# msracver/Relation-Networks-for-Object-Detection

Hardware: AMD Instinct MI355X
Metric: images/sec (1000x600, 300 ROIs) (higher is better)
Workload: dtype bf16; 1 GPU; BASELINE configs[1]: ResNet-101 Faster-RCNN + 2 relation modules (N=300, 16 heads, d=1024) + soft-NMS(0.6) + top-100, 600x1000 images, 300 proposals, random-init weights; launch=hipGraph replay, batches_in_flight=1, parallelism=replicas x1 (no data-path collective), ranks_seen_by_rccl=1

## Files before the change

### include/relnet_hip.h

```cpp
#ifndef RELNET_HIP_H
#define RELNET_HIP_H

#ifdef __cplusplus
extern "C" {
#endif

enum { RELNET_F32 = 0, RELNET_BF16 = 1 };

int relnet_version(void);
const char* relnet_last_error(void);
unsigned long long relnet_stream_capture_id(void* stream);

void _nms(int* keep_out, int* num_out, const float* boxes_host, int boxes_num, int boxes_dim,
          float nms_overlap_thresh, int device_id);

int relnet_proposal_decode(const float* cls_prob, const long* cls_strides4, const float* deltas,
                           const long* delta_strides4, const float* im_info, const double* base_anchors,
                           float* boxes , float* scores , int B, int A, int h, int w,
                           int feat_stride, int min_size, int softmax_pairs, void* stream);
int relnet_topk_sort(const float* scores, const float* boxes, float* out_boxes5, int* out_index,
                     int* out_count, int B, int n, int K, void* stream);
int relnet_nms_mask(const float* boxes5, const int* counts , unsigned long long* mask,
                    int B, int n, int n_stride, float thresh, void* stream);
int relnet_nms_scan(const unsigned long long* mask, const float* boxes5, const int* counts, float* rois,
// ... 89 lines not shown
                                 int B, int H, int N, int M, int Mpad, float scale, int in_dtype, int out_dtype,
                                 const int* key_count, void* stream);
void relnet_relation_attention_debug_lds_f32(int on);

int relnet_relation_attention_fused(const void* q, long q_ld, long q_bs, const void* k, long k_ld, long k_bs,
                                    const void* vwt, long vwt_ld, long vwt_bs, const float* boxes, int box_stride,
                                    int box_off, const float* wp, const float* bp, const float* divisors8,
                                    const float* bout, const void* resid, long resid_ld, long resid_bs, void* out,
                                    long out_ld, long out_bs, void* out_act, long act_ld, long act_bs, int B, int H,
                                    int N, int M, int Mpad, float scale, void* stream);

int relnet_bottleneck_chain(const void* mid2, const void* x, const void* w3f, const void* w1f, const float* b3,
                            const float* b1, void* x_next, void* mid1_next, long P, int mid, void* stream);
int relnet_bottleneck_chain_proj(const void* mid2, const void* x_in, const void* w3f, const void* wpf, const void* w1f,
                                 const float* b3p, const float* b1, void* x_next, void* mid1_next, long P, int mid, void* stream);

int relnet_conv3x3_c64(const void* in, const void* w_frag, const float* bias, int relu, void* out, int B, int H, int W,
                       void* stream);


int relnet_pack_w_frag(const void* w, long ldw, void* out, int N, int K, void* stream);
int relnet_conv2d_nhwc_wf(const void* in, long in_pix, long in_img, const void* w, const void* w_frag, const float* bias,
                          const void* resid, int relu, void* out, long ldc, int B, int H, int W, int Cin, int Cout, int R,
                          int S, int stride, int dil, int pad, int out_dtype, void* stream);

int relnet_detect_head(const float* cls_score, long cs_ld, const float* bbox_pred, long bp_ld, const float* rois,
                       const float* im_info, float* cls_prob, double* boxes, int R, int C, int rois_per_image,
                       int delta_off, void* stream);
int relnet_detect_head_ex(const float* cls_score, long cs_ld, const float* bbox_pred, long bp_ld, const float* rois,
                          const float* im_info, float* cls_prob, double* boxes, int R, int C, int rois_per_image,
                          int delta_off, const int* n_valid, void* stream);
int relnet_class_nms(const float* cls_prob, const double* boxes, double* dets, int* counts, int B, int N, int C,
                     float score_thresh, double nms_param, int soft, int max_picks, void* stream);
// ... 227 lines not shown
```

### relation-networks-for-object-detection_amd/backbone.py

```python
import math
import os

import torch
import torch.nn.functional as F

from . import ops

UNITS = (3, 4, 23, 3)
FILTERS = (256, 512, 1024, 2048)
EPS = 1e-5
PIXEL_MEANS = (103.06, 115.90, 123.15)


def unit_names(fpn=False):
    out = []
    in_ch = 64
    for si, (n, oc) in enumerate(zip(UNITS, FILTERS)):
        stage = si + 2
        for u in range(n):
            if n <= 3 or stage == 2 or stage == 5:
                name = 'abc'[u]
            else:
                name = 'a' if u == 0 else 'b%d' % u
            stride = 2 if (u == 0 and (stage in (3, 4) or (fpn and stage == 5))) else 1
# ... 67 lines not shown


class Backbone(object):

    def __init__(self, params, dtype=torch.bfloat16, device='cuda', channels_last=True, impl=None, stem='hip', dcn=False,
                 fpn=False, chain=True, frozen_only=False, pixel_means=PIXEL_MEANS):
        self.dtype, self.device, self.dcn, self.fpn = dtype, device, dcn, fpn
        self.frozen_only = frozen_only
        self.pixel_means = tuple(float(v) for v in pixel_means)
        self.use_chain = chain
        env = os.environ.get('RELNET_STAGE_SPLIT')
        if env not in (None, '', '0'):
            self.stage_split = {int(a): int(b) for a, b in (kv.split(':') for kv in env.split(','))}
        if os.environ.get('RELNET_INPLACE_EXPAND') is not None:
            self.inplace_expand = os.environ['RELNET_INPLACE_EXPAND'] not in ('', '0')
        self.impl = impl or ('hip' if dtype == torch.bfloat16 else ('hip32' if dtype == torch.float32 and torch.device(device).type == 'cuda' else 'miopen'))
        if self.impl == 'hip' and torch.device(device).type == 'cuda':
            ops.asm_selfcheck()
        self.stem = stem
        assert self.impl in ('hip', 'hip32', 'miopen') and (self.impl != 'hip' or dtype == torch.bfloat16) and (self.impl != 'hip32' or dtype == torch.float32)
        self.mf = torch.channels_last if channels_last else torch.contiguous_format
        self.w = {}
        self.wp = {}
        self.wf = {}
        self.b32 = {}
        self.wp32 = {}
        for conv, bn, oc, ic, k in conv_bn_names():
            if frozen_only and not conv.startswith(('conv1', 'res2')):
                continue
            w, b = fold_bn(params[conv + '_weight'], params[bn + '_gamma'], params[bn + '_beta'],
# ... 90 lines not shown
    def _forward_hip(self, data, rpn_hook=None, im_info=None):
        if self.stem == 'hip':
            x = ops.stem_fused(data, self.w_stem, self.b32['conv1'], im_info, self.pixel_means)
        elif self.stem == 'hip3':
            x = ops.stem_conv7(self._float_image(data, im_info, torch.float32), self.w_stem, self.b32['conv1'], relu=True)
            x = ops.stem_bias_relu_pool(x, self.zero_bias64)
        else:
            x = self._float_image(data, im_info, torch.float32).to(self.dtype).contiguous(memory_format=self.mf)
            x = F.conv2d(x, self.w['conv1'][0], None, stride=2, padding=3)
            x = ops.stem_bias_relu_pool(x.permute(0, 2, 3, 1), self.b32['conv1'])
        conv4 = None
        ends = {}
        y_next = None
        side, hooked = None, None
        self.last_chain_units, self.last_side_stream, self.last_stage_split = [], False, {}
        ui = 0
        while ui < len(self.units):
            unit = self.units[ui]
            stage, proj = unit[0], unit[7]
            if stage == 5 and conv4 is None:
                conv4 = x
                if rpn_hook is not None and not self.fpn:
                    main = torch.cuda.current_stream()
                    side = self._side_stream()
                    self.last_side_stream = True
                    side.wait_stream(main)
                    with torch.cuda.stream(side):
                        hooked = self._rpn_head(conv4)
                        hooked = hooked + (rpn_hook(hooked[0], hooked[1]),)
            if proj and stage > 2:
                ends[stage - 1] = x
            nsplit = self._stage_split(stage, x, unit) if proj else 1
            if nsplit > 1:
                stage_units = [u for u in self.units if u[0] == stage]
                x = self._run_stage_split(x, stage_units, nsplit)
                ui += len(stage_units)
                continue
            x, y_next = self._unit_hip(x, unit, y_next, inplace=self.inplace_expand)
            ui += 1
        conv5 = x
        nchw = lambda t: t.permute(0, 3, 1, 2)
        if self.fpn:
            tops = {32: self._hconv(conv5, 'fpn_ft32_1x1')}
            for lvl, src in ((16, ends[4]), (8, ends[3]), (4, ends[2])):
                tops[lvl] = ops.upsample2x_add_(self._hconv(src, 'fpn_ft%d_1x1' % lvl), tops[lvl * 2])
            out = {'fpn_ft%d' % lvl: nchw(self._hconv(tops[lvl], 'fpn_ft%d_3x3' % lvl, pad=1)) for lvl in (4, 8, 16, 32)}
            out.update(conv4=nchw(conv4), conv5=nchw(conv5))
            return out
        feat = self._hconv(conv5, 'conv_new_1', relu=True)
        out = dict(conv4=nchw(conv4), conv5=nchw(conv5), conv_new_1_relu=nchw(feat))
        if hooked is not None:
            torch.cuda.current_stream().wait_stream(side)
            out.update(rpn_cls_score=hooked[0], rpn_bbox_pred=hooked[1], rpn_hook=hooked[2])
        else:
            out['rpn_cls_score'], out['rpn_bbox_pred'] = self._rpn_head(conv4)
        return out

    stage_split = None
    inplace_expand = True

    def _stage_split(self, stage, x, unit):
        return int(self.stage_split.get(stage, 1)) if self.stage_split else 1

    def _run_stage_split(self, x, stage_units, nsplit):
        B = x.shape[0]
        stage = stage_units[0][0]
        st, nm, ic, mc, oc, stride, dil, proj = stage_units[0]
        Ho, Wo = (x.shape[1] - 1) // stride + 1, (x.shape[2] - 1) // stride + 1
        out = torch.empty((B, Ho, Wo, oc), device=x.device, dtype=x.dtype)
        bounds = [(B * i) // nsplit for i in range(nsplit + 1)]
        self.last_stage_split[stage] = [hi - lo for lo, hi in zip(bounds, bounds[1:])]
        for lo, hi in zip(bounds, bounds[1:]):
            xs, ys = x[lo:hi], None
            for unit in stage_units:
                xs, ys = self._unit_hip(xs, unit, ys, sc_out=out[lo:hi] if unit[7] else None, inplace=self.inplace_expand, force_chain=True)
            if xs.data_ptr() != out[lo:hi].data_ptr():
                out[lo:hi].copy_(xs)
        return out

    def _unit_hip(self, x, unit, y_pre=None, sc_out=None, inplace=False, force_chain=False):
        stage, nm, ic, mc, oc, stride, dil, proj = unit
        fuse_proj = (nm in self.chain_proj and sc_out is None and x.is_contiguous()
                     and (force_chain or ops.chain_worthwhile(x.numel() // x.shape[-1], mc)))
        if fuse_proj:
            sc = None
        elif proj:
            w, b, k = self.wp['res%s_branch1' % nm]
            sc = ops.conv2d_nhwc(x, w, b, ksize=k, stride=stride, out=sc_out)
        else:
            sc = x
        y = y_pre if y_pre is not None else self._hconv(x, 'res%s_branch2a' % nm, stride=stride, relu=True)
        if self.dcn and stage == 5:
            y = self._deform_2b(y.permute(0, 3, 1, 2), 'res%s_branch2b' % nm,
                                self._hconv(y, 'res%s_branch2b_offset' % nm, pad=2, dil=2, out_dtype=torch.float32).permute(0, 3, 1, 2))
            y = y.permute(0, 2, 3, 1)
        elif ('res%s_branch2b' % nm) in self.halo3:
# ... 117 lines not shown
```

### relation-networks-for-object-detection_amd/csrc/bottleneck.hip

```cpp
#include "common.h"

namespace relnet {

typedef const __attribute__((address_space(1))) void* gas_ptr;
typedef __attribute__((address_space(3))) void* las_ptr;

__device__ __forceinline__ void chain_glds16(const void* src, unsigned lds_byte_addr) {
  asm volatile("s_mov_b32 m0, %1\n\ts_nop 0\n\tglobal_load_lds_dwordx4 %0, off" ::"v"(src), "s"(lds_byte_addr) : "memory", "m0");
}

struct ChainArgs {
  const unsigned short* m2;
  const unsigned short* x;
  const uint4* w3f;
  const uint4* w1f;
  const float* b3;
  const float* b1;
  const unsigned short* xin;
  const uint4* wpf;
  unsigned short* xn;
  unsigned short* m1;
  int P;
  int dbg;
};

template <int MID, bool STREAM, bool REDUCE = true, int KSPLIT = 1, bool PROJ = false>
__global__ __launch_bounds__(512) void bottleneck_chain_kernel(ChainArgs a) {
  static_assert(!PROJ || (!STREAM && KSPLIT == 1), "the projection form exists for the resident-weight kernel");
  static_assert(KSPLIT == 1 || (STREAM && !REDUCE), "k-split passes exist for the streamed expand-only form");
  constexpr int COUT = 4 * MID, KS = MID / 16, KSS = KS / KSPLIT, RT = MID / 32, NP = COUT / 64;
  static_assert(!REDUCE || MID <= 128, "MID = 256 with the second product is chain256_roles_kernel");
  constexpr int W3P = 2 * KSS * 1024, W1P = REDUCE ? 4 * RT * 1024 : 0;
  constexpr int WPP = PROJ ? W3P : 0;
  constexpr int PASSB = W3P + WPP + W1P;
  constexpr int STG = PROJ ? 4096 : 8192;
  constexpr int WBYTES = STREAM ? 2 * PASSB : NP * PASSB;
  extern __shared__ __attribute__((aligned(16))) unsigned char smem[];
  const int tid = threadIdx.x, lane = tid & 63;
  const int wave = __builtin_amdgcn_readfirstlane(tid >> 6);
  const int half = lane >> 5, l31 = lane & 31;
  unsigned char* stage = smem + WBYTES + wave * STG;
  float* sB3 = (float*)(smem + WBYTES + 8 * STG);
  float* sB1 = sB3 + COUT;
  for (int i = tid; i < COUT; i += 512) sB3[i] = a.b3[i];
  if constexpr (REDUCE) for (int i = tid; i < MID; i += 512) sB1[i] = a.b1[i];
  if constexpr (!STREAM) {
    for (int i = tid; i < NP * PASSB / 16; i += 512) {
      const int p = i / (PASSB / 16), r = i % (PASSB / 16);
      uint4 v;
      if (r < W3P / 16) v = a.w3f[(long)p * (W3P / 16) + r];
      else if (r < (W3P + WPP) / 16) v = a.wpf[(long)p * (W3P / 16) + (r - W3P / 16)];
      else { const int q = (r - (W3P + WPP) / 16) >> 6, rt = q >> 2, kk = q & 3; v = a.w1f[((long)rt * (COUT / 16) + p * 4 + kk) * 64 + (r & 63)]; }
      ((uint4*)smem)[i] = v;
    }
  }
  __syncthreads();
  const int ntile = (a.P + 31) / 32;
  const int drow = lane >> 3, dslot = lane & 7;
  auto issue_x = [&](int p0, int p) {
    if constexpr (PROJ) return;
    unsigned char* sb = stage + (p & 1) * 4096;
#pragma unroll
    for (int i = 0; i < 4; ++i) {
      const int row = 8 * i + drow;
      const unsigned off = ((unsigned)min(p0 + row, a.P - 1) * COUT + p * 64 + ((dslot ^ ((row >> 1) & 7)) << 3)) * 2u;
      __builtin_amdgcn_global_load_lds((gas_ptr)((const unsigned char*)a.x + off), (las_ptr)(sb + i * 1024), 16, 0, 0);
    }
  };
  auto issue_w = [&](int st) {
    if constexpr (STREAM) {
      const int p = st / KSPLIT, kh = st % KSPLIT;
      unsigned char* wb = smem + (st & 1) * PASSB;
#pragma unroll
      for (int i = 0; i < (2 * KSS + (REDUCE ? 4 * RT : 0)) / 8; ++i) {
        const int q = wave + 8 * i;
        if (q < 2 * KSS) {
          const int ct = q / KSS, ks = q % KSS;
          __builtin_amdgcn_global_load_lds((gas_ptr)(a.w3f + ((long)((p * 2 + ct) * KS + kh * KSS + ks) * 64 + lane)), (las_ptr)(wb + q * 1024), 16, 0, 0);
        } else {
          const int q1 = q - 2 * KSS, rt = q1 >> 2, kk = q1 & 3;
// ... 6 lines not shown
    const unsigned char* sb = stage + (PROJ ? 0 : (p & 1) * 4096) + lane * 16;
    const uint4 v0 = *(const uint4*)sb, v1 = *(const uint4*)(sb + 1024), v2 = *(const uint4*)(sb + 2048), v3 = *(const uint4*)(sb + 3072);
    asm volatile("s_waitcnt lgkmcnt(0)" ::: "memory");
    auto put = [&](int i, const uint4& v) {
      const int row = 8 * i + drow;
      if (p0 + row < a.P) *(uint4*)((unsigned char*)a.xn + ((unsigned)(p0 + row) * COUT + p * 64 + ((dslot ^ ((row >> 1) & 7)) << 3)) * 2u) = v;
    };
    put(0, v0); put(1, v1); put(2, v2); put(3, v3);
  };

  const int t_first = blockIdx.x * 8 + wave;
  const int t_step = gridDim.x * 8;
  const int n_iter = STREAM ? ((ntile + 7) / 8 - (int)blockIdx.x + (int)gridDim.x - 1) / (int)gridDim.x
                            : (ntile - t_first + t_step - 1) / t_step;
  if (n_iter <= 0) return;
  issue_x(t_first * 32, 0);
  issue_w(0);
  for (int it = 0; it < n_iter; ++it) {
    const int p0 = (t_first + it * t_step) * 32;
    const int px = min(p0 + l31, a.P - 1);
    bf16x8 m2f[KS];
#pragma unroll
    for (int ks = 0; ks < KS; ++ks) m2f[ks] = *(const bf16x8*)(a.m2 + (long)px * MID + 16 * ks + 8 * half);
    bf16x8 xf[PROJ ? KS : 1];
    if constexpr (PROJ) {
#pragma unroll
      for (int ks = 0; ks < KS; ++ks) xf[ks] = *(const bf16x8*)(a.xin + (long)px * MID + 16 * ks + 8 * half);
    }
    f32x16 m1acc[RT];
#pragma unroll
    for (int rt = 0; rt < RT; ++rt)
#pragma unroll
      for (int r = 0; r < 16; ++r) m1acc[rt][r] = 0.f;
#pragma unroll 1
    for (int p = 0; p < NP; ++p) {
      f32x16 acc[2];
#pragma unroll
      for (int kh = 0; kh < KSPLIT; ++kh) {
        const int st = p * KSPLIT + kh;
        if constexpr (STREAM) asm volatile("s_waitcnt vmcnt(0)\n\ts_barrier" ::: "memory");
        else if constexpr (!PROJ) asm volatile("s_waitcnt vmcnt(0)" ::: "memory");
        if (kh == 0) {
          if (!PROJ && p > 0) flush(p0, p - 1);
          if (p + 1 < NP) issue_x(p0, p + 1);
          else if (it + 1 < n_iter) issue_x(p0 + t_step * 32, 0);
        }
        if (st + 1 < NP * KSPLIT) issue_w(st + 1);
        else if (it + 1 < n_iter) issue_w(0);
        const uint4* w3 = (const uint4*)(smem + (STREAM ? (st & 1) : st) * PASSB);
#pragma unroll
        for (int ct = 0; ct < 2; ++ct) {
          if (kh == 0)
#pragma unroll
            for (int r = 0; r < 16; ++r) acc[ct][r] = 0.f;
#pragma unroll
          for (int ks = 0; ks < KSS; ++ks)
            acc[ct] = __builtin_amdgcn_mfma_f32_32x32x16_bf16(*(const bf16x8*)&w3[(ct * KSS + ks) * 64 + lane], m2f[kh * KSS + ks], acc[ct], 0, 0, 0);
          if constexpr (PROJ) {
            const uint4* wp = (const uint4*)((const unsigned char*)w3 + W3P);
#pragma unroll
// ... 260 lines not shown
using namespace relnet;

static int g_chain_dbg = 0;
extern "C" void relnet_chain_debug(int flags) { g_chain_dbg = flags; }

extern "C" int relnet_bottleneck_chain(const void* mid2, const void* x, const void* w3f, const void* w1f, const float* b3,
                                       const float* b1, void* x_next, void* mid1_next, long P, int mid, void* stream) {
  RELNET_REQUIRE(mid2 && x && w3f && b3 && x_next, "relnet_bottleneck_chain: null operand");
  RELNET_REQUIRE((w1f && b1 && mid1_next) || (!w1f && !b1 && !mid1_next), "relnet_bottleneck_chain: w1f, b1 and mid1_next are given together (or all NULL: expand + shortcut + ReLU only)");
  RELNET_REQUIRE(mid == 64 || mid == 128 || mid == 256 || (mid == 512 && !mid1_next), "relnet_bottleneck_chain: mid = %d unsupported (64, 128, 256; 512 without the reduce product)", mid);
  RELNET_REQUIRE(P > 0 && P * 8 * mid < (1L << 32), "relnet_bottleneck_chain: bad pixel count %ld (the 4 mid-channel map must stay below 4 GiB)", P);
  ChainArgs a;
  a.m2 = (const unsigned short*)mid2; a.x = (const unsigned short*)x; a.w3f = (const uint4*)w3f; a.w1f = (const uint4*)w1f;
  a.b3 = b3; a.b1 = b1; a.xn = (unsigned short*)x_next; a.m1 = (unsigned short*)mid1_next; a.P = (int)P;
  a.xin = nullptr; a.wpf = nullptr; a.dbg = g_chain_dbg;
  static relnet::PerDeviceOnce attr_once;
  if (attr_once.first()) {
    hipFuncSetAttribute((const void*)bottleneck_chain_kernel<64, false>, hipFuncAttributeMaxDynamicSharedMemorySize, 160 * 1024);
    hipFuncSetAttribute((const void*)bottleneck_chain_kernel<128, true>, hipFuncAttributeMaxDynamicSharedMemorySize, 160 * 1024);
    hipFuncSetAttribute((const void*)bottleneck_chain_kernel<64, false, false>, hipFuncAttributeMaxDynamicSharedMemorySize, 160 * 1024);
    hipFuncSetAttribute((const void*)bottleneck_chain_kernel<128, true, false>, hipFuncAttributeMaxDynamicSharedMemorySize, 160 * 1024);
    hipFuncSetAttribute((const void*)bottleneck_chain_kernel<256, true, false>, hipFuncAttributeMaxDynamicSharedMemorySize, 160 * 1024);
    hipFuncSetAttribute((const void*)bottleneck_chain_kernel<512, true, false, 2>, hipFuncAttributeMaxDynamicSharedMemorySize, 160 * 1024);
    hipFuncSetAttribute((const void*)chain256_roles_kernel, hipFuncAttributeMaxDynamicSharedMemorySize, 160 * 1024);
  }
  const long ntile = (P + 31) / 32;
  const unsigned grid = (unsigned)(ntile < 8 * 256 ? (ntile + 7) / 8 : 256);
  const size_t lds = 65536  + 65536  + (size_t)5 * mid * 4;
  if (mid1_next) {
    if (mid == 64) bottleneck_chain_kernel<64, false><<<grid, 512, lds, (hipStream_t)stream>>>(a);
    else if (mid == 128) bottleneck_chain_kernel<128, true><<<grid, 512, lds, (hipStream_t)stream>>>(a);
    else {
      const long nset = (ntile + 3) / 4;
      chain256_roles_kernel<<<(unsigned)(nset < 256 ? nset : 256), 512, relnet::kRolesLdsBytes, (hipStream_t)stream>>>(a);
    }
  } else {
    if (mid == 64) bottleneck_chain_kernel<64, false, false><<<grid, 512, lds, (hipStream_t)stream>>>(a);
    else if (mid == 128) bottleneck_chain_kernel<128, true, false><<<grid, 512, lds, (hipStream_t)stream>>>(a);
    else if (mid == 256) bottleneck_chain_kernel<256, true, false><<<grid, 512, lds, (hipStream_t)stream>>>(a);
    else bottleneck_chain_kernel<512, true, false, 2><<<grid, 512, lds, (hipStream_t)stream>>>(a);
  }
  return check_launch("relnet_bottleneck_chain");
}

extern "C" int relnet_bottleneck_chain_proj(const void* mid2, const void* x_in, const void* w3f, const void* wpf, const void* w1f,
                                            const float* b3p, const float* b1, void* x_next, void* mid1_next, long P, int mid,
                                            void* stream) {
  RELNET_REQUIRE(mid2 && x_in && w3f && wpf && b3p && x_next, "relnet_bottleneck_chain_proj: null operand");
  RELNET_REQUIRE((w1f && b1 && mid1_next) || (!w1f && !b1 && !mid1_next), "relnet_bottleneck_chain_proj: w1f, b1 and mid1_next are given together (or all NULL)");
  RELNET_REQUIRE(mid == 64, "relnet_bottleneck_chain_proj: mid = %d unsupported (64)", mid);
  RELNET_REQUIRE(P > 0 && P * 8 * mid < (1L << 32), "relnet_bottleneck_chain_proj: bad pixel count %ld (x_next is addressed with 32-bit byte offsets: the 4 mid-channel map must stay below 4 GiB)", P);
  ChainArgs a;
  a.m2 = (const unsigned short*)mid2; a.x = nullptr; a.w3f = (const uint4*)w3f; a.w1f = (const uint4*)w1f;
  a.b3 = b3p; a.b1 = b1; a.xn = (unsigned short*)x_next; a.m1 = (unsigned short*)mid1_next; a.P = (int)P;
  a.xin = (const unsigned short*)x_in; a.wpf = (const uint4*)wpf; a.dbg = 0;
  static relnet::PerDeviceOnce attr_once;
  if (attr_once.first()) {
    hipFuncSetAttribute((const void*)bottleneck_chain_kernel<64, false, true, 1, true>, hipFuncAttributeMaxDynamicSharedMemorySize, 160 * 1024);
    hipFuncSetAttribute((const void*)bottleneck_chain_kernel<64, false, false, 1, true>, hipFuncAttributeMaxDynamicSharedMemorySize, 160 * 1024);
  }
  const long ntile = (P + 31) / 32;
  const unsigned grid = (unsigned)(ntile < 8 * 256 ? (ntile + 7) / 8 : 256);
  const size_t lds = (size_t)4 * (8192 + 8192 + (mid1_next ? 8192 : 0)) + 8 * 4096 + (size_t)5 * mid * 4;
  if (mid1_next) bottleneck_chain_kernel<64, false, true, 1, true><<<grid, 512, lds, (hipStream_t)stream>>>(a);
  else bottleneck_chain_kernel<64, false, false, 1, true><<<grid, 512, lds, (hipStream_t)stream>>>(a);
  return check_launch("relnet_bottleneck_chain_proj");
}

namespace relnet {

__device__ __attribute__((aligned(16))) const unsigned int g_zero_chunk[4] = {0u, 0u, 0u, 0u};

struct Halo3Args {
  const unsigned short* in;
  const uint4* wf;
  const float* bias;
  unsigned short* out;
  int B, H, W, relu;
  int tiles_x, tiles_y;
};

constexpr int kHaloW = 34, kHaloSlots = 40;
constexpr int kHaloBytes = 10 * kHaloSlots * 128;

__global__ __launch_bounds__(512) void conv3x3_c64_halo_kernel(Halo3Args a) {
  extern __shared__ __attribute__((aligned(16))) unsigned char smem[];
  unsigned char* sOut = smem + 2 * kHaloBytes;
  const int tid = threadIdx.x, lane = tid & 63;
  const int wave = __builtin_amdgcn_readfirstlane(tid >> 6);
  const int half = lane >> 5, l31 = lane & 31;
  const int chh = wave & 1, rg = wave >> 1;
  bf16x8 wfrag[36];
#pragma unroll
  for (int ks = 0; ks < 36; ++ks) wfrag[ks] = *(const bf16x8*)&a.wf[(chh * 36 + ks) * 64 + lane];
  float* sBias = (float*)(sOut + 32768);
  if (tid < 64) sBias[tid] = a.bias[tid];
  const int per_img = a.tiles_x * a.tiles_y;
  const int ntile = a.B * per_img;

  auto issue_halo = [&](int t, unsigned char* buf) {
    asm volatile("" : "+s"(t));
    const int b = t / per_img, ty = (t % per_img) / a.tiles_x, tx = t % a.tiles_x;
    const int y0 = ty * 8 - 1, x0 = tx * 32 - 1;
    const unsigned short* img = a.in + (long)b * a.H * a.W * 64;
    int ln = lane;
    asm volatile("" : "+v"(ln));
    const int r8 = ln >> 3, slot = ln & 7;
#pragma unroll
    for (int i = 0; i < 7; ++i) {
      const int j = wave + 8 * i;
      if (j >= 50) break;
      const int hy = j / 5, part = j - 5 * hy;
      const int y = y0 + hy, hx = part * 8 + r8, x = x0 + hx;
      const int sw = (4 * (hy + part) + (r8 >> 1)) & 7;
      const bool ok = hx < kHaloW && y >= 0 && y < a.H && x >= 0 && x < a.W;
      const void* src = ok ? (const void*)(img + ((long)y * a.W + x) * 64 + ((slot ^ sw) << 3)) : (const void*)g_zero_chunk;
      __builtin_amdgcn_global_load_lds((gas_ptr)src, (las_ptr)(buf + j * 1024), 16, 0, 0);
    }
  };

  int t = blockIdx.x;
  if (t < ntile) issue_halo(t, smem);
  asm volatile("s_waitcnt vmcnt(0)\n\ts_barrier" ::: "memory");
  int cur = 0;
  for (; t < ntile; t += gridDim.x, cur ^= 1) {
    const int tn = t + gridDim.x;
    if (tn < ntile) issue_halo(tn, smem + (cur ^ 1) * kHaloBytes);
    const unsigned char* hb = smem + cur * kHaloBytes;
    int lq = l31;
    asm volatile("" : "+v"(lq));
    f32x16 acc[2];
#pragma unroll
    for (int rr = 0; rr < 2; ++rr)
#pragma unroll
      for (int r = 0; r < 16; ++r) acc[rr][r] = 0.f;
    {
      auto frag = [&](int s_, int rr) -> bf16x8 {
        const int tap = s_ >> 2, kb = s_ & 3, dy = tap / 3, dx = tap % 3;
        const int hp = (2 * rg + rr + dy) * kHaloSlots + lq + dx;
        return *(const bf16x8*)(hb + hp * 128 + (((2 * kb + half) ^ ((hp >> 1) & 7)) << 4));
      };
      bf16x8 pq[3][2];
      pq[0][0] = frag(0, 0); pq[0][1] = frag(0, 1);
      pq[1][0] = frag(1, 0); pq[1][1] = frag(1, 1);
#pragma unroll
      for (int s_ = 0; s_ < 36; ++s_) {
        if (s_ + 2 < 36) { pq[(s_ + 2) % 3][0] = frag(s_ + 2, 0); pq[(s_ + 2) % 3][1] = frag(s_ + 2, 1); }
        acc[0] = __builtin_amdgcn_mfma_f32_32x32x16_bf16(wfrag[s_], pq[s_ % 3][0], acc[0], 0, 0, 0);
        acc[1] = __builtin_amdgcn_mfma_f32_32x32x16_bf16(wfrag[s_], pq[s_ % 3][1], acc[1], 0, 0, 0);
        __builtin_amdgcn_sched_barrier(0);
      }
    }
#pragma unroll
    for (int rr = 0; rr < 2; ++rr) {
      const int p = (2 * rg + rr) * 32 + l31;
#pragma unroll
      for (int g = 0; g < 4; ++g) {
        const float4 bq = *(const float4*)(sBias + chh * 32 + 8 * g + 4 * half);
        float v[4] = {acc[rr][4 * g] + bq.x, acc[rr][4 * g + 1] + bq.y, acc[rr][4 * g + 2] + bq.z, acc[rr][4 * g + 3] + bq.w};
#pragma unroll
        for (int e = 0; e < 4; ++e) v[e] = a.relu ? fmaxf(v[e], 0.f) : v[e];
        *(uint2*)(sOut + p * 128 + (((chh * 4 + g) ^ ((p >> 1) & 7)) << 4) + 8 * half) = make_uint2(pack_bf16x2(v[0], v[1]), pack_bf16x2(v[2], v[3]));
      }
    }
    asm volatile("s_waitcnt lgkmcnt(0)\n\ts_barrier" ::: "memory");
    {
      const int b = t / per_img, ty = (t % per_img) / a.tiles_x, tx = t % a.tiles_x;
      unsigned short* img = a.out + (long)b * a.H * a.W * 64;
      const unsigned char* so = sOut + wave * 4096 + lane * 16;
      const uint4 v0 = *(const uint4*)so, v1 = *(const uint4*)(so + 1024), v2 = *(const uint4*)(so + 2048), v3 = *(const uint4*)(so + 3072);
      asm volatile("s_waitcnt vmcnt(0) lgkmcnt(0)" ::: "memory");
      auto put = [&](int i, const uint4& v) {
        const int p = 8 * (wave * 4 + i) + (lane >> 3), slot = lane & 7;
        const int y = ty * 8 + (p >> 5), x = tx * 32 + (p & 31);
        if (y < a.H && x < a.W) *(uint4*)(img + ((long)y * a.W + x) * 64 + ((slot ^ ((p >> 1) & 7)) << 3)) = v;
      };
      put(0, v0); put(1, v1); put(2, v2); put(3, v3);
    }
    __builtin_amdgcn_s_barrier();
  }
}

}

extern "C" int relnet_conv3x3_c64(const void* in, const void* w_frag, const float* bias, int relu, void* out, int B, int H,
                                  int W, void* stream) {
  RELNET_REQUIRE(in && w_frag && bias && out, "relnet_conv3x3_c64: null operand");
  RELNET_REQUIRE(B > 0 && H > 0 && W > 0 && (long)B * H * W < (1L << 31), "relnet_conv3x3_c64: bad geometry B=%d H=%d W=%d", B, H, W);
  Halo3Args a;
  a.in = (const unsigned short*)in; a.wf = (const uint4*)w_frag; a.bias = bias; a.out = (unsigned short*)out;
  a.B = B; a.H = H; a.W = W; a.relu = relu;
  a.tiles_x = (W + 31) / 32; a.tiles_y = (H + 7) / 8;
  static relnet::PerDeviceOnce attr_once;
  if (attr_once.first()) {
    hipFuncSetAttribute((const void*)conv3x3_c64_halo_kernel, hipFuncAttributeMaxDynamicSharedMemorySize, 160 * 1024);
  }
  const long ntile = (long)B * a.tiles_x * a.tiles_y;
  const unsigned grid = (unsigned)(ntile < 256 ? ntile : 256);
  conv3x3_c64_halo_kernel<<<grid, 512, 2 * kHaloBytes + 32768 + 256, (hipStream_t)stream>>>(a);
  return check_launch("relnet_conv3x3_c64");
}
```

### relation-networks-for-object-detection_amd/lib.py

```python
import ctypes as C
import os
import sys

HERE = os.path.dirname(os.path.abspath(__file__))
LIB_PATH = os.environ.get('RELNET_LIB') or os.path.join(HERE, 'librelnet_hip.so')

F32, BF16 = 0, 1


class RelnetError(RuntimeError):
    pass


_lib = None

_vp, _i, _l, _f, _d = C.c_void_p, C.c_int, C.c_long, C.c_float, C.c_double

_SIGNATURES = {
    'relnet_version': (C.c_int, []),
    'relnet_last_error': (C.c_char_p, []),
    'relnet_gemm_nt': (C.c_int, [_vp, _l, _l, _vp, _l, _l, _vp, _l, _l, _vp, _i, _vp, _i,
                                 _i, _i, _i, _i, _i, _i, _vp]),
    'relnet_geometry_bias': (C.c_int, [_vp, _i, _i, _vp, _vp, _vp, _vp, _i, _vp, _vp, _i, _i, _i, _i,
                                       _i, _i, _vp]),
    'relnet_relation_attention': (C.c_int, [_vp, _l, _l, _vp, _l, _l, _vp, _l, _l, _vp, _i, _l, _vp,
                                            _vp, _l, _l, _vp, _l, _l, _vp, _l, _l, _vp,
                                            _i, _i, _i, _i, _i, _f, _i, _i, _vp]),
    'relnet_relation_attention_kc': (C.c_int, [_vp, _l, _l, _vp, _l, _l, _vp, _l, _l, _vp, _i, _l, _vp,
                                               _vp, _l, _l, _vp, _l, _l, _vp, _l, _l, _vp,
                                               _i, _i, _i, _i, _i, _f, _i, _i, _vp, _vp]),
    'relnet_relation_attention_fused': (C.c_int, [_vp, _l, _l, _vp, _l, _l, _vp, _l, _l, _vp, _i, _i, _vp, _vp, _vp,
                                                  _vp, _vp, _l, _l, _vp, _l, _l, _vp, _l, _l,
                                                  _i, _i, _i, _i, _i, _f, _vp]),
    'relnet_bottleneck_chain': (C.c_int, [_vp, _vp, _vp, _vp, _vp, _vp, _vp, _vp, _l, _i, _vp]),
    'relnet_bottleneck_chain_proj': (C.c_int, [_vp, _vp, _vp, _vp, _vp, _vp, _vp, _vp, _vp, _l, _i, _vp]),
    'relnet_conv3x3_c64': (C.c_int, [_vp, _vp, _vp, _i, _vp, _i, _i, _i, _vp]),
    'relnet_proposal_decode': (C.c_int, [_vp, _vp, _vp, _vp, _vp, _vp, _vp, _vp, _i, _i, _i, _i, _i, _i, _i, _vp]),
    'relnet_topk_sort': (C.c_int, [_vp, _vp, _vp, _vp, _vp, _i, _i, _i, _vp]),
    'relnet_nms_mask': (C.c_int, [_vp, _vp, _vp, _i, _i, _i, _f, _vp]),
    'relnet_nms_scan': (C.c_int, [_vp, _vp, _vp, _vp, _vp, _vp, _vp, _i, _i, _i, _i, _i, _i, _vp]),
    '_nms': (None, [_vp, _vp, _vp, _i, _i, _f, _i]),
    'relnet_roi_pool_fwd': (C.c_int, [_vp, _vp, _vp, _vp, _vp, _vp, _i, _i, _i, _i, _i, _i, _f, _i, _i, _vp]),
    'relnet_roi_align_fwd': (C.c_int, [_vp, _vp, _vp, _vp, _vp, _i, _i, _i, _i, _i, _i, _f, _i, _i, _i, _i, _vp]),
    'relnet_roi_align_bwd': (C.c_int, [_vp, _vp, _vp, _vp, _vp, _i, _i, _i, _i, _i, _i, _f, _i, _i, _i, _i, _vp]),
    'relnet_roi_align_levels_fwd': (C.c_int, [_vp, _vp, _vp, _vp, _vp, _i, _vp, _vp, _vp, _vp] + [_i] * 9 + [_vp]),
    'relnet_roi_align_levels_bwd': (C.c_int, [_vp, _vp, _vp, _vp, _vp, _vp, _vp, _vp, _vp] + [_i] * 10 + [_vp]),
    'relnet_roi_pool_bwd': (C.c_int, [_vp, _vp, _vp, _vp, _vp, _l, _l, _i, _i, _i, _i, _i, _i, _i, _vp]),
    'relnet_roi_pool_bwd_ex': (C.c_int, [_vp, _vp, _vp, _vp, _vp, _l, _l, _l, _i, _i, _i, _i, _i, _i, _i, _vp]),
    'relnet_roi_pool_fpn_bwd_ex': (C.c_int, [_vp, _vp, _vp, _vp, _vp, _vp, _vp, _vp, _vp, _i, _i, _i, _i, _i, _i, _i, _vp]),
    'relnet_detect_head': (C.c_int, [_vp, _l, _vp, _l, _vp, _vp, _vp, _vp, _i, _i, _i, _i, _vp]),
    'relnet_detect_head_ex': (C.c_int, [_vp, _l, _vp, _l, _vp, _vp, _vp, _vp, _i, _i, _i, _i, _vp, _vp]),
# ... 167 lines not shown
```

### relation-networks-for-object-detection_amd/ops.py

```python
import math
import os

import torch

from . import lib as _lib

F32, BF16 = _lib.F32, _lib.BF16


def _dt(t):
    if t.dtype == torch.float32:
        return F32
    if t.dtype == torch.bfloat16:
        return BF16
    raise TypeError("unsupported dtype %s (float32 or bfloat16)" % t.dtype)


def _chk(*ts):
    for t in ts:
        if t is not None:
            if not t.is_cuda:
                raise _lib.RelnetError("relnet ops need GPU tensors (HIP kernels only; no CPU fallback)")


# ... 517 lines not shown


HALO3_CHANNELS = (64,)


def conv3x3_halo(x, w_frag, bias, relu=True):
    _chk(x, w_frag, bias)
    B, H, W, C = x.shape
    assert C in HALO3_CHANNELS and x.is_contiguous() and x.dtype == torch.bfloat16 and bias.dtype == torch.float32
    assert w_frag.numel() == 9 * C * C
    out = torch.empty_like(x)
    _lib.call('relnet_conv3x3_c%d' % C, x.data_ptr(), w_frag.data_ptr(), bias.data_ptr(), int(relu), out.data_ptr(), B, H, W, _stream())
    return out


def conv3x3_c64(x, w_frag, bias, relu=True):
    return conv3x3_halo(x, w_frag, bias, relu)


CHAIN_MIDS = (64, 128, 256)
CHAIN_EXPAND_MIDS = (64, 128, 256, 512)


CHAIN_MIN_PIXELS = {64: 16384, 128: 65536, 256: 8192, 512: 49152, 'streamed': 98304}


def chain_worthwhile(pixels, mid):
    return pixels >= CHAIN_MIN_PIXELS[mid if mid in CHAIN_MIN_PIXELS else 'streamed'] and pixels * 8 * mid < (1 << 32)


# ... 10 lines not shown
    return w_packed[row, col].contiguous()


def bottleneck_chain(mid2, x, w3_frag, w1_frag, b3, b1, inplace=False):
    _chk(mid2, x, w3_frag, w1_frag, b3, b1)
    mid = mid2.shape[-1]
    assert mid2.is_contiguous() and x.is_contiguous() and x.shape[-1] == 4 * mid and x.shape[:-1] == mid2.shape[:-1]
    assert mid2.dtype == torch.bfloat16 and x.dtype == torch.bfloat16 and b3.dtype == torch.float32
    assert (w1_frag is None) == (b1 is None) and (b1 is None or b1.dtype == torch.float32)
    assert mid in (CHAIN_MIDS if w1_frag is not None else CHAIN_EXPAND_MIDS)
    xn = x if inplace else torch.empty_like(x)
    m1 = torch.empty_like(mid2) if w1_frag is not None else None
    _lib.call('relnet_bottleneck_chain', mid2.data_ptr(), x.data_ptr(), w3_frag.data_ptr(), _ptr(w1_frag), b3.data_ptr(),
              _ptr(b1), xn.data_ptr(), _ptr(m1), mid2.numel() // mid, mid, _stream())
    return xn, m1


def bottleneck_chain_proj(mid2, x_in, w3_frag, wp_frag, w1_frag, b3p, b1):
    _chk(mid2, x_in, w3_frag, wp_frag, w1_frag, b3p, b1)
    mid = mid2.shape[-1]
    assert mid == 64 and x_in.shape == mid2.shape and mid2.is_contiguous() and x_in.is_contiguous()
    assert mid2.dtype == torch.bfloat16 and x_in.dtype == torch.bfloat16 and b3p.dtype == torch.float32
    assert (w1_frag is None) == (b1 is None)
    xn = torch.empty(mid2.shape[:-1] + (4 * mid,), device=mid2.device, dtype=torch.bfloat16)
    m1 = torch.empty_like(mid2) if w1_frag is not None else None
    _lib.call('relnet_bottleneck_chain_proj', mid2.data_ptr(), x_in.data_ptr(), w3_frag.data_ptr(), wp_frag.data_ptr(), _ptr(w1_frag),
              b3p.data_ptr(), _ptr(b1), xn.data_ptr(), _ptr(m1), mid2.numel() // mid, mid, _stream())
    return xn, m1


# ... 763 lines not shown
```

Before: 2762 images/s.

## Compute only even pixels in the stage-final unit feeding a stride-2 projection

When a bottleneck unit's output is consumed only by the next stage's stride-2 1x1 convolutions (branch1 and branch2a), the unit now computes its 3x3 conv at stride 2. Its expand-plus-residual chain kernel gathers the residual at even pixels only, and the following unit then runs at stride 1. This removes three quarters of the 3x3 and expand work, plus the output writes, for the res2c and res3b3-type units. It adds a stride-2 halo conv3x3 kernel variant and a gather path in the chain kernel, with more complex index math and a different LDS layout.

```diff
diff --git a/include/relnet_hip.h b/include/relnet_hip.h
--- a/include/relnet_hip.h
+++ b/include/relnet_hip.h
@@ -127,9 +127,13 @@
                             const float* b1, void* x_next, void* mid1_next, long P, int mid, void* stream);
 int relnet_bottleneck_chain_proj(const void* mid2, const void* x_in, const void* w3f, const void* wpf, const void* w1f,
                                  const float* b3p, const float* b1, void* x_next, void* mid1_next, long P, int mid, void* stream);
+int relnet_bottleneck_chain_s2(const void* mid2, const void* x, const void* w3f, const float* b3, void* x_next, int B, int H,
+                               int W, int mid, void* stream);
 
 int relnet_conv3x3_c64(const void* in, const void* w_frag, const float* bias, int relu, void* out, int B, int H, int W,
                        void* stream);
+int relnet_conv3x3_c64_s2(const void* in, const void* w_frag, const float* bias, int relu, void* out, int B, int H, int W,
+                          void* stream);
 
 
 int relnet_pack_w_frag(const void* w, long ldw, void* out, int N, int K, void* stream);
diff --git a/relation-networks-for-object-detection_amd/backbone.py b/relation-networks-for-object-detection_amd/backbone.py
--- a/relation-networks-for-object-detection_amd/backbone.py
+++ b/relation-networks-for-object-detection_amd/backbone.py
@@ -105,6 +105,8 @@
             self.stage_split = {int(a): int(b) for a, b in (kv.split(':') for kv in env.split(','))}
         if os.environ.get('RELNET_INPLACE_EXPAND') is not None:
             self.inplace_expand = os.environ['RELNET_INPLACE_EXPAND'] not in ('', '0')
+        if os.environ.get('RELNET_QUARTER_UNITS') is not None:
+            self.quarter_units = os.environ['RELNET_QUARTER_UNITS'] not in ('', '0')
         self.impl = impl or ('hip' if dtype == torch.bfloat16 else ('hip32' if dtype == torch.float32 and torch.device(device).type == 'cuda' else 'miopen'))
         if self.impl == 'hip' and torch.device(device).type == 'cuda':
             ops.asm_selfcheck()
@@ -225,6 +227,8 @@
         y_next = None
         side, hooked = None, None
         self.last_chain_units, self.last_side_stream, self.last_stage_split = [], False, {}
+        self.last_quarter_units = []
+        compact = False
         ui = 0
         while ui < len(self.units):
             unit = self.units[ui]
@@ -247,7 +251,9 @@
                 x = self._run_stage_split(x, stage_units, nsplit)
                 ui += len(stage_units)
                 continue
-            x, y_next = self._unit_hip(x, unit, y_next, inplace=self.inplace_expand)
+            quarter = self._quarter_ok(x, unit, self.units[ui + 1] if ui + 1 < len(self.units) else None)
+            x, y_next = self._unit_hip(x, unit, y_next, inplace=self.inplace_expand, quarter=quarter, subsampled=compact)
+            compact = quarter
             ui += 1
         conv5 = x
         nchw = lambda t: t.permute(0, 3, 1, 2)
@@ -270,6 +276,22 @@
     stage_split = None
     inplace_expand = True
 
+    quarter_units = True
+
+    def _quarter_ok(self, x, unit, nxt):
+        stage, nm, ic, mc, oc, stride, dil, proj = unit
+        if not self.quarter_units or self.fpn or nxt is None or nxt[0] != stage + 1 or nxt[5] != 2 or not nxt[7]:
+            return False
+        ch = self.chain.get(nm)
+        if ch is None or ch[1] is not None or mc not in ops.CHAIN_S2_MIDS or proj or dil != 1 or (self.dcn and stage == 5):
+            return False
+        if mc in ops.HALO3_CHANNELS and ('res%s_branch2b' % nm) not in self.halo3:
+            return False
+        if self.stage_split and (self._stage_split(stage, x, unit) > 1 or self._stage_split(nxt[0], x, nxt) > 1):
+            return False
+        B, H, W, C = x.shape
+        return C == oc and x.numel() * 2 < (1 << 32) and ops.chain_worthwhile(B * ((H - 1) // 2 + 1) * ((W - 1) // 2 + 1), mc)
+
     def _stage_split(self, stage, x, unit):
         return int(self.stage_split.get(stage, 1)) if self.stage_split else 1
 
@@ -289,8 +311,22 @@
                 out[lo:hi].copy_(xs)
         return out
 
-    def _unit_hip(self, x, unit, y_pre=None, sc_out=None, inplace=False, force_chain=False):
+    def _unit_hip(self, x, unit, y_pre=None, sc_out=None, inplace=False, force_chain=False, quarter=False, subsampled=False):
         stage, nm, ic, mc, oc, stride, dil, proj = unit
+        if subsampled:
+            assert stride == 2 and proj
+            stride = 1
+        if quarter:
+            y = y_pre if y_pre is not None else self._hconv(x, 'res%s_branch2a' % nm, relu=True)
+            if ('res%s_branch2b' % nm) in self.halo3:
+                y = ops.conv3x3_halo_s2(y.contiguous(), *self.halo3['res%s_branch2b' % nm], relu=True)
+            else:
+                y = self._hconv(y, 'res%s_branch2b' % nm, stride=2, pad=1, relu=True)
+            w3f, _, b3, _ = self.chain[nm]
+            if nm not in self.last_chain_units:
+                self.last_chain_units.append(nm)
+            self.last_quarter_units.append(nm)
+            return ops.bottleneck_chain_s2(y, x.contiguous(), w3f, b3), None
         fuse_proj = (nm in self.chain_proj and sc_out is None and x.is_contiguous()
                      and (force_chain or ops.chain_worthwhile(x.numel() // x.shape[-1], mc)))
         if fuse_proj:
diff --git a/relation-networks-for-object-detection_amd/csrc/bottleneck.hip b/relation-networks-for-object-detection_amd/csrc/bottleneck.hip
--- a/relation-networks-for-object-detection_amd/csrc/bottleneck.hip
+++ b/relation-networks-for-object-detection_amd/csrc/bottleneck.hip
@@ -21,12 +21,14 @@
   unsigned short* xn;
   unsigned short* m1;
   int P;
+  int H, W, Ho, Wo;
   int dbg;
 };
 
-template <int MID, bool STREAM, bool REDUCE = true, int KSPLIT = 1, bool PROJ = false>
+template <int MID, bool STREAM, bool REDUCE = true, int KSPLIT = 1, bool PROJ = false, bool GATHER = false>
 __global__ __launch_bounds__(512) void bottleneck_chain_kernel(ChainArgs a) {
   static_assert(!PROJ || (!STREAM && KSPLIT == 1), "the projection form exists for the resident-weight kernel");
+  static_assert(!GATHER || (!REDUCE && !PROJ && KSPLIT == 1), "the stride-2 gather exists for the plain expand-only forms");
   static_assert(KSPLIT == 1 || (STREAM && !REDUCE), "k-split passes exist for the streamed expand-only form");
   constexpr int COUT = 4 * MID, KS = MID / 16, KSS = KS / KSPLIT, RT = MID / 32, NP = COUT / 64;
   static_assert(!REDUCE || MID <= 128, "MID = 256 with the second product is chain256_roles_kernel");
@@ -57,13 +59,26 @@
   __syncthreads();
   const int ntile = (a.P + 31) / 32;
   const int drow = lane >> 3, dslot = lane & 7;
+  unsigned xrow[GATHER ? 4 : 1];
+  auto gather_rows = [&](int p0) {
+    if constexpr (GATHER) {
+      const unsigned hw = (unsigned)(a.Ho * a.Wo);
+#pragma unroll
+      for (int i = 0; i < 4; ++i) {
+        const unsigned q = (unsigned)min(p0 + 8 * i + drow, a.P - 1);
+        const unsigned b = q / hw, r = q - b * hw, yo = r / (unsigned)a.Wo, xo = r - yo * (unsigned)a.Wo;
+        xrow[i] = ((b * (unsigned)a.H + 2u * yo) * (unsigned)a.W + 2u * xo) * (COUT * 2u);
+      }
+    }
+  };
   auto issue_x = [&](int p0, int p) {
     if constexpr (PROJ) return;
     unsigned char* sb = stage + (p & 1) * 4096;
 #pragma unroll
     for (int i = 0; i < 4; ++i) {
       const int row = 8 * i + drow;
-      const unsigned off = ((unsigned)min(p0 + row, a.P - 1) * COUT + p * 64 + ((dslot ^ ((row >> 1) & 7)) << 3)) * 2u;
+      const unsigned off = GATHER ? xrow[i] + (p * 64 + ((dslot ^ ((row >> 1) & 7)) << 3)) * 2u
+                                  : ((unsigned)min(p0 + row, a.P - 1) * COUT + p * 64 + ((dslot ^ ((row >> 1) & 7)) << 3)) * 2u;
       __builtin_amdgcn_global_load_lds((gas_ptr)((const unsigned char*)a.x + off), (las_ptr)(sb + i * 1024), 16, 0, 0);
     }
   };
@@ -100,6 +115,7 @@
   const int n_iter = STREAM ? ((ntile + 7) / 8 - (int)blockIdx.x + (int)gridDim.x - 1) / (int)gridDim.x
                             : (ntile - t_first + t_step - 1) / t_step;
   if (n_iter <= 0) return;
+  gather_rows(t_first * 32);
   issue_x(t_first * 32, 0);
   issue_w(0);
   for (int it = 0; it < n_iter; ++it) {
@@ -129,7 +145,7 @@
         if (kh == 0) {
           if (!PROJ && p > 0) flush(p0, p - 1);
           if (p + 1 < NP) issue_x(p0, p + 1);
-          else if (it + 1 < n_iter) issue_x(p0 + t_step * 32, 0);
+          else if (it + 1 < n_iter) { gather_rows(p0 + t_step * 32); issue_x(p0 + t_step * 32, 0); }
         }
         if (st + 1 < NP * KSPLIT) issue_w(st + 1);
         else if (it + 1 < n_iter) issue_w(0);
@@ -420,6 +436,7 @@
   a.m2 = (const unsigned short*)mid2; a.x = (const unsigned short*)x; a.w3f = (const uint4*)w3f; a.w1f = (const uint4*)w1f;
   a.b3 = b3; a.b1 = b1; a.xn = (unsigned short*)x_next; a.m1 = (unsigned short*)mid1_next; a.P = (int)P;
   a.xin = nullptr; a.wpf = nullptr; a.dbg = g_chain_dbg;
+  a.H = a.W = a.Ho = a.Wo = 0;
   static relnet::PerDeviceOnce attr_once;
   if (attr_once.first()) {
     hipFuncSetAttribute((const void*)bottleneck_chain_kernel<64, false>, hipFuncAttributeMaxDynamicSharedMemorySize, 160 * 1024);
@@ -447,6 +464,32 @@
     else bottleneck_chain_kernel<512, true, false, 2><<<grid, 512, lds, (hipStream_t)stream>>>(a);
   }
   return check_launch("relnet_bottleneck_chain");
+}
+
+extern "C" int relnet_bottleneck_chain_s2(const void* mid2, const void* x, const void* w3f, const float* b3, void* x_next, int B,
+                                          int H, int W, int mid, void* stream) {
+  RELNET_REQUIRE(mid2 && x && w3f && b3 && x_next && x_next != x, "relnet_bottleneck_chain_s2: null operand (or x_next == x: this form is never in place)");
+  RELNET_REQUIRE(mid == 64 || mid == 128, "relnet_bottleneck_chain_s2: mid = %d unsupported (64, 128)", mid);
+  RELNET_REQUIRE(B > 0 && H > 0 && W > 0 && (long)B * H * W * 8 * mid < (1L << 32),
+                 "relnet_bottleneck_chain_s2: bad geometry B=%d H=%d W=%d (the full 4 mid-channel map must stay below 4 GiB)", B, H, W);
+  ChainArgs a;
+  a.m2 = (const unsigned short*)mid2; a.x = (const unsigned short*)x; a.w3f = (const uint4*)w3f; a.w1f = nullptr;
+  a.b3 = b3; a.b1 = nullptr; a.xn = (unsigned short*)x_next; a.m1 = nullptr;
+  a.xin = nullptr; a.wpf = nullptr; a.dbg = 0;
+  a.H = H; a.W = W; a.Ho = (H - 1) / 2 + 1; a.Wo = (W - 1) / 2 + 1;
+  const long P = (long)B * a.Ho * a.Wo;
+  a.P = (int)P;
+  static relnet::PerDeviceOnce attr_once;
+  if (attr_once.first()) {
+    hipFuncSetAttribute((const void*)bottleneck_chain_kernel<64, false, false, 1, false, true>, hipFuncAttributeMaxDynamicSharedMemorySize, 160 * 1024);
+    hipFuncSetAttribute((const void*)bottleneck_chain_kernel<128, true, false, 1, false, true>, hipFuncAttributeMaxDynamicSharedMemorySize, 160 * 1024);
+  }
+  const long ntile = (P + 31) / 32;
+  const unsigned grid = (unsigned)(ntile < 8 * 256 ? (ntile + 7) / 8 : 256);
+  const size_t lds = 65536 + 65536 + (size_t)5 * mid * 4;
+  if (mid == 64) bottleneck_chain_kernel<64, false, false, 1, false, true><<<grid, 512, lds, (hipStream_t)stream>>>(a);
+  else bottleneck_chain_kernel<128, true, false, 1, false, true><<<grid, 512, lds, (hipStream_t)stream>>>(a);
+  return check_launch("relnet_bottleneck_chain_s2");
 }
 
 extern "C" int relnet_bottleneck_chain_proj(const void* mid2, const void* x_in, const void* w3f, const void* wpf, const void* w1f,
@@ -460,6 +503,7 @@
   a.m2 = (const unsigned short*)mid2; a.x = nullptr; a.w3f = (const uint4*)w3f; a.w1f = (const uint4*)w1f;
   a.b3 = b3p; a.b1 = b1; a.xn = (unsigned short*)x_next; a.m1 = (unsigned short*)mid1_next; a.P = (int)P;
   a.xin = (const unsigned short*)x_in; a.wpf = (const uint4*)wpf; a.dbg = 0;
+  a.H = a.W = a.Ho = a.Wo = 0;
   static relnet::PerDeviceOnce attr_once;
   if (attr_once.first()) {
     hipFuncSetAttribute((const void*)bottleneck_chain_kernel<64, false, true, 1, true>, hipFuncAttributeMaxDynamicSharedMemorySize, 160 * 1024);
@@ -484,14 +528,21 @@
   unsigned short* out;
   int B, H, W, relu;
   int tiles_x, tiles_y;
+  int Ho, Wo;
 };
 
 constexpr int kHaloW = 34, kHaloSlots = 40;
 constexpr int kHaloBytes = 10 * kHaloSlots * 128;
-
+constexpr int kHalo2Row = 65, kHalo2Even = 33;
+constexpr int kHalo2Dma = (9 * kHalo2Row + 7) / 8;
+constexpr int kHalo2Bytes = kHalo2Dma * 1024;
+
+template <bool S2>
 __global__ __launch_bounds__(512) void conv3x3_c64_halo_kernel(Halo3Args a) {
+  constexpr int NR = S2 ? 1 : 2;
+  constexpr int HB = S2 ? kHalo2Bytes : kHaloBytes;
   extern __shared__ __attribute__((aligned(16))) unsigned char smem[];
-  unsigned char* sOut = smem + 2 * kHaloBytes;
+  unsigned char* sOutDense = smem + 2 * HB;
   const int tid = threadIdx.x, lane = tid & 63;
   const int wave = __builtin_amdgcn_readfirstlane(tid >> 6);
   const int half = lane >> 5, l31 = lane & 31;
@@ -499,7 +550,7 @@
   bf16x8 wfrag[36];
 #pragma unroll
   for (int ks = 0; ks < 36; ++ks) wfrag[ks] = *(const bf16x8*)&a.wf[(chh * 36 + ks) * 64 + lane];
-  float* sBias = (float*)(sOut + 32768);
+  float* sBias = (float*)(smem + 2 * HB + (S2 ? 0 : 32768));
   if (tid < 64) sBias[tid] = a.bias[tid];
   const int per_img = a.tiles_x * a.tiles_y;
   const int ntile = a.B * per_img;
@@ -512,6 +563,22 @@
     int ln = lane;
     asm volatile("" : "+v"(ln));
     const int r8 = ln >> 3, slot = ln & 7;
+    if constexpr (S2) {
+      const int ys = 8 * ty - 1, xs = 64 * tx - 1;
+#pragma unroll
+      for (int i = 0; i < (kHalo2Dma + 7) / 8; ++i) {
+        const int j = wave + 8 * i;
+        if (j >= kHalo2Dma) break;
+        const int q = 8 * j + r8, hy = q / kHalo2Row, sl = q - kHalo2Row * hy;
+        const int hx = sl < kHalo2Even ? 2 * sl : 2 * (sl - kHalo2Even) + 1;
+        const int y = ys + hy, x = xs + hx;
+        const int sw = (4 * j + (r8 >> 1)) & 7;
+        const bool ok = hy < 9 && y >= 0 && y < a.H && x >= 0 && x < a.W;
+        const void* src = ok ? (const void*)(img + ((long)y * a.W + x) * 64 + ((slot ^ sw) << 3)) : (const void*)g_zero_chunk;
+        __builtin_amdgcn_global_load_lds((gas_ptr)src, (las_ptr)(buf + j * 1024), 16, 0, 0);
+      }
+      return;
+    }
 #pragma unroll
     for (int i = 0; i < 7; ++i) {
       const int j = wave + 8 * i;
@@ -531,35 +598,41 @@
   int cur = 0;
   for (; t < ntile; t += gridDim.x, cur ^= 1) {
     const int tn = t + gridDim.x;
-    if (tn < ntile) issue_halo(tn, smem + (cur ^ 1) * kHaloBytes);
-    const unsigned char* hb = smem + cur * kHaloBytes;
+    if (tn < ntile) issue_halo(tn, smem + (cur ^ 1) * HB);
+    const unsigned char* hb = smem + cur * HB;
+    unsigned char* sOut = S2 ? smem + cur * HB : sOutDense;
     int lq = l31;
     asm volatile("" : "+v"(lq));
-    f32x16 acc[2];
-#pragma unroll
-    for (int rr = 0; rr < 2; ++rr)
+    f32x16 acc[NR];
+#pragma unroll
+    for (int rr = 0; rr < NR; ++rr)
 #pragma unroll
       for (int r = 0; r < 16; ++r) acc[rr][r] = 0.f;
     {
       auto frag = [&](int s_, int rr) -> bf16x8 {
         const int tap = s_ >> 2, kb = s_ & 3, dy = tap / 3, dx = tap % 3;
-        const int hp = (2 * rg + rr + dy) * kHaloSlots + lq + dx;
+        const int hp = S2 ? (2 * rg + dy) * kHalo2Row + lq + (dx == 1 ? kHalo2Even : dx >> 1)
+                          : (2 * rg + rr + dy) * kHaloSlots + lq + dx;
         return *(const bf16x8*)(hb + hp * 128 + (((2 * kb + half) ^ ((hp >> 1) & 7)) << 4));
       };
-      bf16x8 pq[3][2];
-      pq[0][0] = frag(0, 0); pq[0][1] = frag(0, 1);
-      pq[1][0] = frag(1, 0); pq[1][1] = frag(1, 1);
+      bf16x8 pq[3][NR];
+#pragma unroll
+      for (int rr = 0; rr < NR; ++rr) { pq[0][rr] = frag(0, rr); pq[1][rr] = frag(1, rr); }
 #pragma unroll
       for (int s_ = 0; s_ < 36; ++s_) {
-        if (s_ + 2 < 36) { pq[(s_ + 2) % 3][0] = frag(s_ + 2, 0); pq[(s_ + 2) % 3][1] = frag(s_ + 2, 1); }
-        acc[0] = __builtin_amdgcn_mfma_f32_32x32x16_bf16(wfrag[s_], pq[s_ % 3][0], acc[0], 0, 0, 0);
-        acc[1] = __builtin_amdgcn_mfma_f32_32x32x16_bf16(wfrag[s_], pq[s_ % 3][1], acc[1], 0, 0, 0);
+        if (s_ + 2 < 36) {
+#pragma unroll
+          for (int rr = 0; rr < NR; ++rr) pq[(s_ + 2) % 3][rr] = frag(s_ + 2, rr);
+        }
+#pragma unroll
+        for (int rr = 0; rr < NR; ++rr) acc[rr] = __builtin_amdgcn_mfma_f32_32x32x16_bf16(wfrag[s_], pq[s_ % 3][rr], acc[rr], 0, 0, 0);
         __builtin_amdgcn_sched_barrier(0);
       }
     }
-#pragma unroll
-    for (int rr = 0; rr < 2; ++rr) {
-      const int p = (2 * rg + rr) * 32 + l31;
+    if constexpr (S2) __builtin_amdgcn_s_barrier();
+#pragma unroll
+    for (int rr = 0; rr < NR; ++rr) {
+      const int p = (NR * rg + rr) * 32 + l31;
 #pragma unroll
       for (int g = 0; g < 4; ++g) {
         const float4 bq = *(const float4*)(sBias + chh * 32 + 8 * g + 4 * half);
@@ -572,16 +645,19 @@
     asm volatile("s_waitcnt lgkmcnt(0)\n\ts_barrier" ::: "memory");
     {
       const int b = t / per_img, ty = (t % per_img) / a.tiles_x, tx = t % a.tiles_x;
-      unsigned short* img = a.out + (long)b * a.H * a.W * 64;
-      const unsigned char* so = sOut + wave * 4096 + lane * 16;
-      const uint4 v0 = *(const uint4*)so, v1 = *(const uint4*)(so + 1024), v2 = *(const uint4*)(so + 2048), v3 = *(const uint4*)(so + 3072);
+      unsigned short* img = a.out + (long)b * a.Ho * a.Wo * 64;
+      const unsigned char* so = sOut + wave * (2048 * NR) + lane * 16;
+      const uint4 v0 = *(const uint4*)so, v1 = *(const uint4*)(so + 1024);
+      uint4 v2 = v0, v3 = v1;
+      if constexpr (NR == 2) { v2 = *(const uint4*)(so + 2048); v3 = *(const uint4*)(so + 3072); }
       asm volatile("s_waitcnt vmcnt(0) lgkmcnt(0)" ::: "memory");
       auto put = [&](int i, const uint4& v) {
-        const int p = 8 * (wave * 4 + i) + (lane >> 3), slot = lane & 7;
-        const int y = ty * 8 + (p >> 5), x = tx * 32 + (p & 31);
-        if (y < a.H && x < a.W) *(uint4*)(img + ((long)y * a.W + x) * 64 + ((slot ^ ((p >> 1) & 7)) << 3)) = v;
+        const int p = 8 * (wave * 2 * NR + i) + (lane >> 3), slot = lane & 7;
+        const int y = ty * 4 * NR + (p >> 5), x = tx * 32 + (p & 31);
+        if (y < a.Ho && x < a.Wo) *(uint4*)(img + ((long)y * a.Wo + x) * 64 + ((slot ^ ((p >> 1) & 7)) << 3)) = v;
       };
-      put(0, v0); put(1, v1); put(2, v2); put(3, v3);
+      put(0, v0); put(1, v1);
+      if constexpr (NR == 2) { put(2, v2); put(3, v3); }
     }
     __builtin_amdgcn_s_barrier();
   }
@@ -596,13 +672,32 @@
   Halo3Args a;
   a.in = (const unsigned short*)in; a.wf = (const uint4*)w_frag; a.bias = bias; a.out = (unsigned short*)out;
   a.B = B; a.H = H; a.W = W; a.relu = relu;
-  a.tiles_x = (W + 31) / 32; a.tiles_y = (H + 7) / 8;
+  a.tiles_x = (W + 31) / 32; a.tiles_y = (H + 7) / 8; a.Ho = H; a.Wo = W;
   static relnet::PerDeviceOnce attr_once;
   if (attr_once.first()) {
-    hipFuncSetAttribute((const void*)conv3x3_c64_halo_kernel, hipFuncAttributeMaxDynamicSharedMemorySize, 160 * 1024);
+    hipFuncSetAttribute((const void*)conv3x3_c64_halo_kernel<false>, hipFuncAttributeMaxDynamicSharedMemorySize, 160 * 1024);
   }
   const long ntile = (long)B * a.tiles_x * a.tiles_y;
   const unsigned grid = (unsigned)(ntile < 256 ? ntile : 256);
-  conv3x3_c64_halo_kernel<<<grid, 512, 2 * kHaloBytes + 32768 + 256, (hipStream_t)stream>>>(a);
+  conv3x3_c64_halo_kernel<false><<<grid, 512, 2 * kHaloBytes + 32768 + 256, (hipStream_t)stream>>>(a);
   return check_launch("relnet_conv3x3_c64");
 }
+
+extern "C" int relnet_conv3x3_c64_s2(const void* in, const void* w_frag, const float* bias, int relu, void* out, int B, int H,
+                                     int W, void* stream) {
+  RELNET_REQUIRE(in && w_frag && bias && out, "relnet_conv3x3_c64_s2: null operand");
+  RELNET_REQUIRE(B > 0 && H > 0 && W > 0 && (long)B * H * W < (1L << 31), "relnet_conv3x3_c64_s2: bad geometry B=%d H=%d W=%d", B, H, W);
+  Halo3Args a;
+  a.in = (const unsigned short*)in; a.wf = (const uint4*)w_frag; a.bias = bias; a.out = (unsigned short*)out;
+  a.B = B; a.H = H; a.W = W; a.relu = relu;
+  a.Ho = (H - 1) / 2 + 1; a.Wo = (W - 1) / 2 + 1;
+  a.tiles_x = (a.Wo + 31) / 32; a.tiles_y = (a.Ho + 3) / 4;
+  static relnet::PerDeviceOnce attr_once;
+  if (attr_once.first()) {
+    hipFuncSetAttribute((const void*)conv3x3_c64_halo_kernel<true>, hipFuncAttributeMaxDynamicSharedMemorySize, 160 * 1024);
+  }
+  const long ntile = (long)B * a.tiles_x * a.tiles_y;
+  const unsigned grid = (unsigned)(ntile < 256 ? ntile : 256);
+  conv3x3_c64_halo_kernel<true><<<grid, 512, 2 * kHalo2Bytes + 256, (hipStream_t)stream>>>(a);
+  return check_launch("relnet_conv3x3_c64_s2");
+}
diff --git a/relation-networks-for-object-detection_amd/lib.py b/relation-networks-for-object-detection_amd/lib.py
--- a/relation-networks-for-object-detection_amd/lib.py
+++ b/relation-networks-for-object-detection_amd/lib.py
@@ -35,6 +35,8 @@
     'relnet_bottleneck_chain': (C.c_int, [_vp, _vp, _vp, _vp, _vp, _vp, _vp, _vp, _l, _i, _vp]),
     'relnet_bottleneck_chain_proj': (C.c_int, [_vp, _vp, _vp, _vp, _vp, _vp, _vp, _vp, _vp, _l, _i, _vp]),
     'relnet_conv3x3_c64': (C.c_int, [_vp, _vp, _vp, _i, _vp, _i, _i, _i, _vp]),
+    'relnet_conv3x3_c64_s2': (C.c_int, [_vp, _vp, _vp, _i, _vp, _i, _i, _i, _vp]),
+    'relnet_bottleneck_chain_s2': (C.c_int, [_vp, _vp, _vp, _vp, _vp, _i, _i, _i, _i, _vp]),
     'relnet_proposal_decode': (C.c_int, [_vp, _vp, _vp, _vp, _vp, _vp, _vp, _vp, _i, _i, _i, _i, _i, _i, _i, _vp]),
     'relnet_topk_sort': (C.c_int, [_vp, _vp, _vp, _vp, _vp, _i, _i, _i, _vp]),
     'relnet_nms_mask': (C.c_int, [_vp, _vp, _vp, _i, _i, _i, _f, _vp]),
diff --git a/relation-networks-for-object-detection_amd/ops.py b/relation-networks-for-object-detection_amd/ops.py
--- a/relation-networks-for-object-detection_amd/ops.py
+++ b/relation-networks-for-object-detection_amd/ops.py
@@ -555,6 +555,16 @@
     return out
 
 
+def conv3x3_halo_s2(x, w_frag, bias, relu=True):
+    _chk(x, w_frag, bias)
+    B, H, W, C = x.shape
+    assert C == 64 and x.is_contiguous() and x.dtype == torch.bfloat16 and bias.dtype == torch.float32
+    assert w_frag.numel() == 9 * C * C
+    out = torch.empty((B, (H - 1) // 2 + 1, (W - 1) // 2 + 1, C), device=x.device, dtype=x.dtype)
+    _lib.call('relnet_conv3x3_c64_s2', x.data_ptr(), w_frag.data_ptr(), bias.data_ptr(), int(relu), out.data_ptr(), B, H, W, _stream())
+    return out
+
+
 def conv3x3_c64(x, w_frag, bias, relu=True):
     return conv3x3_halo(x, w_frag, bias, relu)
 
@@ -595,6 +605,22 @@
     _lib.call('relnet_bottleneck_chain', mid2.data_ptr(), x.data_ptr(), w3_frag.data_ptr(), _ptr(w1_frag), b3.data_ptr(),
               _ptr(b1), xn.data_ptr(), _ptr(m1), mid2.numel() // mid, mid, _stream())
     return xn, m1
+
+
+CHAIN_S2_MIDS = (64, 128)
+
+
+def bottleneck_chain_s2(mid2, x, w3_frag, b3):
+    _chk(mid2, x, w3_frag, b3)
+    mid = mid2.shape[-1]
+    B, H, W, C = x.shape
+    assert mid in CHAIN_S2_MIDS and C == 4 * mid and mid2.shape == (B, (H - 1) // 2 + 1, (W - 1) // 2 + 1, mid)
+    assert mid2.is_contiguous() and x.is_contiguous() and x.numel() * 2 < (1 << 32)
+    assert mid2.dtype == torch.bfloat16 and x.dtype == torch.bfloat16 and b3.dtype == torch.float32
+    xn = torch.empty(mid2.shape[:-1] + (C,), device=x.device, dtype=x.dtype)
+    _lib.call('relnet_bottleneck_chain_s2', mid2.data_ptr(), x.data_ptr(), w3_frag.data_ptr(), b3.data_ptr(), xn.data_ptr(), B, H, W, mid,
+              _stream())
+    return xn
 
 
 def bottleneck_chain_proj(mid2, x_in, w3_frag, wp_frag, w1_frag, b3p, b1):
```

Measured after the change: 2860 images/s, median of 6. +3.5%, better.
